# inferrna/Core

Hardware: AMD Instinct MI355X
Metric: Mrays/s (primary+shadow), 1M-tri scene (higher is better)
Workload: dtype f32

## Files before the change

core_amd/csrc/yk_device.hip:

```cpp
#include <hip/hip_runtime.h>

#include <algorithm>
#include <atomic>
#include <climits>
#include <chrono>
#include <cmath>
#include <cstdio>
#include <cstdlib>
#include <cstring>
#include <mutex>
#include <type_traits>
#include <stdexcept>
#include <string>
#include <thread>
#include <vector>

#include "../../include/yk_api.h"
#include "../../include/yk_test_hooks.h"
#include "../../include/yk_test_hooks_light.h"
#include "photon_map.h"
#include "scene.h"
#include "yk_internal.h"
#include "yk_math.h"

// ... 1780 lines not shown
  if (hit) s_q[off + __popcll(hm & ((1ull << lane) - 1ull))] = (int)threadIdx.x;
  __syncthreads();
  const bool valid = (int)threadIdx.x < tot;
  src = valid ? s_q[threadIdx.x] : 0;
  return valid;
}

enum : uint8_t { SL_TRACED = 1, SL_ADDS = 2 };
struct Batch;
__device__ __forceinline__ long long slot_of(const Batch& B, long long c, int k);
enum : int { PH_HIT = 1, PH_DIFFUSE = 2, PH_LIGHT = 4 };
enum : int { PS_ALIVE = 1, PS_RESOLVE = 2, PS_CONT = 4, PS_EST = 8, PS_EMIT = 256 };

struct Batch {
  int* prim_hit;
  unsigned* soffs;
  float* col;
  float* alpha;
  yk_ray* p_rays;
  yk_hit* p_hits;
  float* thr;
  float* pathcol;
  float* scol_next;
  float* wlast;
  float* emit_b;
  int* pstate;
  int* lsel;
  int* q_owner[2];
  yk_ray* q_rays[2];
  yk_hit* q_hits[2];
  float4* s_dir;
  int split;
  uint8_t* s_occl;
  unsigned* s_idx;
  float* sl_contrib;
  uint8_t* sl_flags;
  float4* samples;
  float2* sxy;
  char4* pext;
  int K;
  long long cap;
  long long kstride;
// ... 1 lines not shown
  long long slot_base;
  const unsigned long long* mq_words;
  int mq_region;
  unsigned* psample;
  uint8_t* incl;
  uint8_t* caus;
  float* emit0;
  int ts;
  float* s_filt;
  float* sl_aux;
};
__device__ __forceinline__ long long slot_of(const Batch& B, long long c, int k) {
  return B.slot_base + (long long)k * B.kstride + c;
}

struct RenderConst {
  int ps;
  int multipass;
  int pass_off;
  int spec;
  int trace_caustics;
  int rdepth;
  int level;
  int spp;
  int nsub;
  int bounces;
  int integrator;
  int transp_bg;
  int nlights;
  int has_bg;
// ... 51 lines not shown
    int lo = 0, hi = TL.ntiles - 1;
    while (lo < hi) {
      const int mid = (lo + hi + 1) >> 1;
      if (TL.base[mid] <= c) lo = mid;
      else hi = mid - 1;
    }
    const int4 T = TL.tiles[lo];
    const long long local = c - TL.base[lo];
    s = (int)((unsigned)local % (unsigned)R.spp);
    const int pl = (int)((unsigned)local / (unsigned)R.spp);
    j = T.x + pl % T.z;
    i = T.y + pl / T.z;
  }
  const unsigned so = fnv32a((unsigned)i * fnv32a((unsigned)j));
  const unsigned psample = (unsigned)(R.pass_off + s);
  B.soffs[c] = so;
  if (R.ps) B.psample[c] = psample;
  float dx = 0.5f, dy = 0.5f;
  if (R.multipass) {
    dx = ri_vdc(psample, so);
    dy = ri_s(psample, so);
  } else if (R.spp > 1) {
    dx = (0.5f + (float)s) * R.d1;
    dy = ri_lp((unsigned)s + so, 0u);
  }
  B.sxy[c] = make_float2(dx, dy);
  const float px = (float)j + dx, py = (float)i + dy;
  const v3 vr = ld3(c_cam.vright), vu = ld3(c_cam.vup), vt = ld3(c_cam.vto), cz = ld3(c_cam.camZ);
  v3 d = vadd(vadd(vmul(px, vr), vmul(py, vu)), vt);
  d = vnormalize_cam(d);
  const v3 from = ld3(c_cam.pos);
// ... 230 lines not shown
}

__device__ __forceinline__ void flush_shadow(const Batch& B, long long c, int kend, int nr, unsigned base,
                                             unsigned long long traced) {
  if (nr == 0) return;
  unsigned r = base;
  for (int k = 0; k < kend; ++k) {
    const long long slot = slot_of(B, c, k);
    const bool t = k < 64 ? ((traced >> k) & 1ull) != 0ull : (B.sl_flags[slot] & SL_TRACED) != 0;
    if (t) B.s_idx[r++] = B.split ? ((unsigned)k << B.kshift) | (unsigned)(B.slot_base + c) : (unsigned)slot;
  }
}

template <bool DIFF = false>
__device__ __forceinline__ yk_ray path_first_segment(const Batch& B, const RenderConst& R, long long c,
                                                     const SurfPt& sp, const DMat& M, v3 dir, int isub) {
  const unsigned s = R.ps ? B.psample[c] : (unsigned)c % (unsigned)R.spp;
  const unsigned offs = (unsigned)(R.nsub * (int)s) + B.soffs[c] + (unsigned)isub;
  const float s1 = ri_vdc(offs, 0u);
  const float s2 = (float)scr_halton(2, offs);
  float pdf, W = B.wlast[c];
  bool ok;
  v3 pdir = V3(0.f, 0.f, 0.f);
  c3 scol = mat_sample<DIFF>(M, sp, vneg(dir), pdir, s1, s2, BSDF_DIFFUSE | BSDF_REFLECT | BSDF_TRANSMIT, pdf, W, ok);
  B.wlast[c] = W;
  scol = cscale(W, scol);
  B.thr[3 * c] = scol.r;
  B.thr[3 * c + 1] = scol.g;
  B.thr[3 * c + 2] = scol.b;
  yk_ray r;
  put_ray(r, sp.P, pdir, YK_MIN_RAYDIST, -1.0f);
  return r;
}

template <bool DIFF, bool XL>
__global__ void __launch_bounds__(YK_PRIMARY_BLOCK) k_shade_primary(DScene S, Batch B, RenderConst R, long long nc,
                                                       unsigned long long* __restrict__ qword) {
  __shared__ DMat s_mats[kMaxMats];
  {
    const int nw = S.nmats * (int)(sizeof(DMat) / sizeof(int));
// ... 17 lines not shown
      const v3 from = V3(r.from[0], r.from[1], r.from[2]), dir = V3(r.dir[0], r.dir[1], r.dir[2]);
      const SurfPt sp = make_surface(S, from, dir, h);
      const DMat& M = s_mats[sp.mat];
      const v3 wo = vneg(dir);
      ph = PH_HIT;
      if (M.flags & BSDF_EMIT) {
        const c3 e = mat_emit(M, sp, wo, true);
        if (R.spec && R.integrator != YK_INTEGRATOR_PHOTON && M.type == YK_MAT_LIGHT) em = e;
        else col = cadd(col, e);
        if (R.integrator == YK_INTEGRATOR_PHOTON && !R.pm_showmap) col = cadd(col, mat_emit(M, sp, wo, false));
        if (M.type == YK_MAT_LIGHT) ph |= PH_LIGHT;
      }
      if (M.flags & BSDF_DIFFUSE) ph |= PH_DIFFUSE;
      if ((M.flags & BSDF_DIFFUSE) && !R.pm_showmap) {
        const unsigned s = R.ps ? B.psample[c] : (unsigned)c % (unsigned)R.spp;
        int k0 = 0;
        for (int l = 0; l < R.nlights; ++l) {
          nr += gen_light<DIFF, XL>(B, c, k0, l, sp, wo, s, B.soffs[c], (unsigned)l, traced, s_mats);
          k0 += c_lights[l].nslots;
        }
        kend = k0;
        if (nr) put_org(B, c, sp.P);
        if (R.integrator == YK_INTEGRATOR_PATH) {
          B.wlast[c] = 0.f;
          seg = path_first_segment<DIFF>(B, R, c, sp, M, dir, 0);
          emit = true;
          if (R.spec) {
            B.incl[c] = 0;
            B.caus[c] = 0;
          }
        }
      }
      alpha = 1.0f;
    } else if (R.has_bg) {
      col = cadd(col, C3(R.bg[0], R.bg[1], R.bg[2]));
    }
    B.prim_hit[c] = ph;
    B.col[3 * c] = col.r;
    B.col[3 * c + 1] = col.g;
    B.col[3 * c + 2] = col.b;
    B.alpha[c] = alpha;
    if (R.spec) {
      B.emit0[3 * c] = em.r;
      B.emit0[3 * c + 1] = em.g;
      B.emit0[3 * c + 2] = em.b;
    }
    if (!R.merged) {
      B.pathcol[3 * c] = 0.f;
      B.pathcol[3 * c + 1] = 0.f;
      B.pathcol[3 * c + 2] = 0.f;
    }
    if (!emit) B.wlast[c] = 0.f;
  }
  unsigned sbase, q;
  wave_append2<YK_PRIMARY_APPEND_WAVE>(qword, valid ? (unsigned)nr : 0u, emit ? 1u : 0u, sbase, q);
  if (valid) flush_shadow(B, c, kend, nr, sbase, traced);
  if (emit) {
    st_ray(&B.q_rays[1][q], seg);
    B.q_owner[1][q] = (int)c;
  }
}

__device__ __forceinline__ c3 slot_value_ts(const Batch& B, long long slot, int kind, c3 lcol, bool spot = false) {
  const c3 a = get_contrib(B, slot);
  const float4 x = *reinterpret_cast<const float4*>(B.sl_aux + 4 * slot);
  const c3 sc = C3(B.s_filt[3 * slot], B.s_filt[3 * slot + 1], B.s_filt[3 * slot + 2]);
  if (kind == 0) {
// ... 52 lines not shown
  B.col[3 * c + 2] = B.col[3 * c + 2] + dl.b;
}

template <bool DIFF>
__global__ void __launch_bounds__(YK_BOUNCE_BLOCK) k_path_start(DScene S, Batch B, RenderConst R, long long nc, int isub,
                                                    unsigned long long* __restrict__ qword) {
  const long long c = (long long)blockIdx.x * blockDim.x + threadIdx.x;
  const bool valid = c < nc;
  bool emit = false;
  yk_ray r;
  if (valid && (B.prim_hit[c] & PH_DIFFUSE)) {
    const yk_hit h = B.p_hits[c];
    const yk_ray pr = B.p_rays[c];
    const v3 from = V3(pr.from[0], pr.from[1], pr.from[2]), dir = V3(pr.dir[0], pr.dir[1], pr.dir[2]);
    const SurfPt sp = make_surface(S, from, dir, h);
    r = path_first_segment<DIFF>(B, R, c, sp, c_mats[sp.mat], dir, isub);
    emit = true;
    if (R.spec) {
      B.incl[c] = 0;
      B.caus[c] = 0;
    }
  }
  unsigned sbase, q;
  wave_append2<YK_BOUNCE_APPEND_WAVE>(qword, 0u, emit ? 1u : 0u, sbase, q);
  if (emit) {
    st_ray(&B.q_rays[1][q], r);
    B.q_owner[1][q] = (int)c;
  }
}

template <bool DIFF, bool XL>
// ... 6 lines not shown
  if (qb >= nq) return;
  unsigned qpre = 0;
  if (B.mq_words)
    for (int r = 0; r < B.mq_region; ++r) qpre += (unsigned)B.mq_words[r];
  long long qi = qb + threadIdx.x;
  bool valid = qi < nq;
  {
    const int prim = valid ? B.q_hits[qin][qi].prim : 0;
    if (valid && prim < 0) {
      const long long c = B.q_owner[qin][qi];
      if (R.spec && depth >= 2 && B.caus[c] && R.has_bg) {
        B.pathcol[3 * c] = B.pathcol[3 * c] + B.thr[3 * c] * R.bg[0];
        B.pathcol[3 * c + 1] = B.pathcol[3 * c + 1] + B.thr[3 * c + 1] * R.bg[1];
        B.pathcol[3 * c + 2] = B.pathcol[3 * c + 2] + B.thr[3 * c + 2] * R.bg[2];
      }
      B.pstate[c] = 0;
    }
    int src;
    valid = pack_block<bounce_block(DIFF)>(valid && prim >= 0, src);
    qi = qb + src;
  }
  const long long c = valid ? B.q_owner[qin][qi] : 0;
  int nr = 0, kend = 0;
  unsigned long long traced = 0;
  bool emit_next = false;
  yk_ray nxt;
  if (valid) {
    const yk_hit h = B.q_hits[qin][qi];
    {
      const yk_ray pr = B.q_rays[qin][qi];
      const v3 from = V3(pr.from[0], pr.from[1], pr.from[2]), dir = V3(pr.dir[0], pr.dir[1], pr.dir[2]);
      const SurfPt sp = make_surface(S, from, dir, h);
      const DMat& M = c_mats[sp.mat];
      const v3 pwo = vneg(dir);
      const unsigned s = R.ps ? B.psample[c] : (unsigned)c % (unsigned)R.spp;
      const unsigned offs = (unsigned)(R.nsub * (int)s) + B.soffs[c] + (unsigned)isub;
      int ps = PS_RESOLVE;
      if ((depth == 1 || (M.flags & BSDF_DIFFUSE)) && R.nlights > 0) {
        Halton h2;
        hal_start(h2, 2u, (unsigned)((int)offs - 1));
        int lnum = (int)(hal_next(h2) * (float)R.nlights);
        if (lnum > R.nlights - 1) lnum = R.nlights - 1;
        if (R.nlights == 1) nr = gen_light<DIFF, XL>(B, c, 0, 0, sp, pwo, s, B.soffs[c], 0u, traced);
        else nr = gen_light<DIFF, XL>(B, c, 0, lnum, sp, pwo, s, B.soffs[c], (unsigned)lnum, traced);
        kend = c_lights[lnum].nslots;
        if (nr) put_org(B, c, sp.P);
        if (R.nlights > 1) B.lsel[c] = lnum;
        ps |= PS_EST;
      }
      c3 em = C3(0.f, 0.f, 0.f);
      bool emits = false;
      if (depth == 1 && (M.flags & BSDF_EMIT)) {
        em = mat_emit(M, sp, pwo, false);
        emits = true;
      }
      if (R.spec && depth >= 2 && B.caus[c] && (M.flags & BSDF_SPECULAR)) {
        em = mat_emit(M, sp, pwo, true);
        emits = true;
      }
      if (emits) {
        B.emit_b[3 * c] = em.r;
        B.emit_b[3 * c + 1] = em.g;
        B.emit_b[3 * c + 2] = em.b;
        ps |= PS_EMIT;
      }
      if (depth < R.bounces) {
        const float s1 = (float)scr_halton(4 * depth + 3, offs);
        const float s2 = (float)scr_halton(4 * depth + 4, offs);
        float pdf, W = B.wlast[c];
        bool ok;
        v3 ndir = dir;
        unsigned sfl;
        c3 sc = mat_sample<DIFF>(M, sp, pwo, ndir, s1, s2, BSDF_ALL, pdf, W, ok, sfl);
        B.wlast[c] = W;
        sc = cscale(W, sc);
        if (!cblack(sc)) {
          if (R.spec) {
            const uint8_t caustic =
                (R.trace_caustics && (sfl & (BSDF_SPECULAR | BSDF_GLOSSY | BSDF_FILTER))) ? 1 : 0;
            B.caus[c] = caustic;
            B.incl[c] = caustic;
          }
          put_ray(nxt, sp.P, ndir, YK_MIN_RAYDIST, -1.0f);
          emit_next = true;
          B.scol_next[3 * c] = sc.r;
          B.scol_next[3 * c + 1] = sc.g;
          B.scol_next[3 * c + 2] = sc.b;
          ps |= PS_CONT;
        }
      }
      B.pstate[c] = ps;
    }
  }
  unsigned sbase, qn;
  wave_append2<YK_BOUNCE_APPEND_WAVE>(qword, valid ? (unsigned)nr : 0u, emit_next ? 1u : 0u, sbase, qn);
  if (valid) flush_shadow(B, c, kend, nr, sbase + qpre, traced);
  if (emit_next) {
    st_ray(&B.q_rays[qin ^ 1][qn], nxt);
    B.q_owner[qin ^ 1][qn] = (int)c;
  }
}

inline auto shade_primary_fn(bool diff, bool xl) {
  return xl ? (diff ? k_shade_primary<true, true> : k_shade_primary<false, true>)
            : (diff ? k_shade_primary<true, false> : k_shade_primary<false, false>);
}
inline auto shade_bounce_fn(bool diff, bool xl) {
  return xl ? (diff ? k_shade_bounce<true, true> : k_shade_bounce<false, true>)
            : (diff ? k_shade_bounce<true, false> : k_shade_bounce<false, false>);
}

__global__ void __launch_bounds__(256) k_resolve_bounce(Batch B, RenderConst R,
                                                        const unsigned long long* __restrict__ qin_word, int depth,
                                                        int qin) {
  const long long nq = (long long)(*qin_word >> 32);
  const long long qi = (long long)blockIdx.x * blockDim.x + threadIdx.x;
  if (qi >= nq) return;
  const long long c = B.q_owner[qin][qi];
  const int ps = B.pstate[c];
  if (!(ps & PS_RESOLVE)) return;
  c3 lcol = C3(0.f, 0.f, 0.f);
  if (ps & PS_EST) {
    const int lnum = R.nlights > 1 ? B.lsel[c] : 0;
    lcol = cscale((float)R.nlights, resolve_light(B, c, 0, lnum));
  }
  if ((depth == 1 || R.spec) && (ps & PS_EMIT))
    lcol = cadd(lcol, C3(B.emit_b[3 * c], B.emit_b[3 * c + 1], B.emit_b[3 * c + 2]));
  const c3 thr = C3(B.thr[3 * c], B.thr[3 * c + 1], B.thr[3 * c + 2]);
  B.pathcol[3 * c] = B.pathcol[3 * c] + lcol.r * thr.r;
  B.pathcol[3 * c + 1] = B.pathcol[3 * c + 1] + lcol.g * thr.g;
  B.pathcol[3 * c + 2] = B.pathcol[3 * c + 2] + lcol.b * thr.b;
  if (ps & PS_CONT) {
    B.thr[3 * c] = thr.r * B.scol_next[3 * c];
    B.thr[3 * c + 1] = thr.g * B.scol_next[3 * c + 1];
    B.thr[3 * c + 2] = thr.b * B.scol_next[3 * c + 2];
    B.pstate[c] = PS_ALIVE;
  } else {
    B.pstate[c] = 0;
  }
}


__host__ __device__ inline Batch merged_region(Batch B, int depth) {
  B.slot_base = (long long)depth * B.cap;
  B.mq_region = depth;
  if (depth >= 1) {
    const long long o = (long long)(depth - 1) * B.cap;
    B.pstate += o;
    B.lsel += o;
    B.emit_b += 3 * o;
    B.scol_next += 3 * o;
  }
  return B;
}

__global__ void __launch_bounds__(256) k_resolve_merged(Batch B, RenderConst R, long long nc, int bounces) {
  const long long c = (long long)blockIdx.x * blockDim.x + threadIdx.x;
  if (c >= nc) return;
  c3 col = C3(B.col[3 * c], B.col[3 * c + 1], B.col[3 * c + 2]);
  if (!(B.prim_hit[c] & PH_DIFFUSE)) {
    B.samples[c] = make_float4(col.r, col.g, col.b, B.alpha[c]);
    return;
  }
  {
    c3 dl = C3(0.f, 0.f, 0.f);
    int k0 = 0;
    for (int l = 0; l < R.nlights; ++l) {
      dl = cadd(dl, resolve_light(B, c, k0, l));
      k0 += c_lights[l].nslots;
    }
    col = C3(col.r + dl.r, col.g + dl.g, col.b + dl.b);
  }
  c3 thr = C3(B.thr[3 * c], B.thr[3 * c + 1], B.thr[3 * c + 2]);
  c3 pc = C3(0.f, 0.f, 0.f);
  for (int depth = 1; depth <= bounces; ++depth) {
    const Batch Bd = merged_region(B, depth);
    const int ps = Bd.pstate[c];
    if (!(ps & PS_RESOLVE)) break;
    c3 lcol = C3(0.f, 0.f, 0.f);
    if (ps & PS_EST) {
      const int lnum = R.nlights > 1 ? Bd.lsel[c] : 0;
      lcol = cscale((float)R.nlights, resolve_light(Bd, c, 0, lnum));
    }
    if (depth == 1 && (ps & PS_EMIT))
      lcol = cadd(lcol, C3(Bd.emit_b[3 * c], Bd.emit_b[3 * c + 1], Bd.emit_b[3 * c + 2]));
    pc = C3(pc.r + lcol.r * thr.r, pc.g + lcol.g * thr.g, pc.b + lcol.b * thr.b);
    if (!(ps & PS_CONT)) break;
    thr = C3(thr.r * Bd.scol_next[3 * c], thr.g * Bd.scol_next[3 * c + 1], thr.b * Bd.scol_next[3 * c + 2]);
  }
  const float ns = (float)R.nsub;
  col = cadd(col, C3(pc.r / ns, pc.g / ns, pc.b / ns));
  B.samples[c] = make_float4(col.r, col.g, col.b, B.alpha[c]);
}

__global__ void __launch_bounds__(256) k_finish(Batch B, RenderConst R, long long nc) {
  const long long c = (long long)blockIdx.x * blockDim.x + threadIdx.x;
  if (c >= nc) return;
  c3 col = C3(B.col[3 * c], B.col[3 * c + 1], B.col[3 * c + 2]);
  if (R.integrator == YK_INTEGRATOR_PATH && (B.prim_hit[c] & PH_DIFFUSE)) {
    const float ns = (float)R.nsub;
    col = cadd(col, C3(B.pathcol[3 * c] / ns, B.pathcol[3 * c + 1] / ns, B.pathcol[3 * c + 2] / ns));
  }
  B.samples[c] = make_float4(col.r, col.g, col.b, B.alpha[c]);
// ... 6 lines not shown
  float* E;
  float* D;
  float* P;
  int* flags;
  int* child;
  float* rcol;
  float* alpha;
  yk_ray* ray;
  unsigned* soffs;
  unsigned* psample;
  unsigned long long* count;
  long long cap;
  int* overflow;
  float* malpha;
};

__global__ void __launch_bounds__(256) k_finish_spec(Batch B, RenderConst R, NodeStore NS, long long base,
                                                     long long n) {
  const long long i = (long long)blockIdx.x * blockDim.x + threadIdx.x;
  if (i >= n) return;
  const long long node = base + i;
  const int ph = B.prim_hit[i];
  const bool loop = R.integrator == YK_INTEGRATOR_PATH && (ph & PH_DIFFUSE);
  c3 P = C3(0.f, 0.f, 0.f);
  if (loop) {
    const float ns = (float)R.nsub;
    P = C3(B.pathcol[3 * i] / ns, B.pathcol[3 * i + 1] / ns, B.pathcol[3 * i + 2] / ns);
  }
  int f = 0;
  if (ph & PH_HIT) f |= NF_HIT;
// ... 40 lines not shown
  mat_specular(M, sp, vneg(dir), refl, refr, d, col);
  const bool want[2] = {refl, refr};
#pragma unroll
  for (int k = 0; k < 2; ++k) {
    if (!want[k]) continue;
    const unsigned long long id = atomicAdd(NS.count, 1ull);
    if ((long long)id >= NS.cap) {
      *NS.overflow = 1;
      continue;
    }
    NS.child[2 * node + k] = (int)id;
    NS.rcol[6 * node + 3 * k] = col[k].r;
    NS.rcol[6 * node + 3 * k + 1] = col[k].g;
    NS.rcol[6 * node + 3 * k + 2] = col[k].b;
    put_ray(NS.ray[id], sp.P, d[k], YK_MIN_RAYDIST, -1.0f);
    NS.soffs[id] = B.soffs[i];
    NS.psample[id] = B.psample[i];
  }
}

__global__ void __launch_bounds__(256) k_fold(Batch B, RenderConst R, NodeStore NS, long long nc) {
  const long long c = (long long)blockIdx.x * blockDim.x + threadIdx.x;
  if (c >= nc) return;
  constexpr int kMaxLevel = 22;
  int nodes[kMaxLevel], stage[kMaxLevel];
  c3 acc[kMaxLevel];
  float alp[kMaxLevel];
  const bool pt = R.integrator == YK_INTEGRATOR_PATH, pm = R.integrator == YK_INTEGRATOR_PHOTON;
  const float a_init = R.transp_bg ? 0.f : 1.f;
  float result_alpha = 0.f;
  bool e = true;
// ... 313 lines not shown
  DBuf() = default;
  DBuf(const DBuf&) = delete;
  DBuf& operator=(const DBuf&) = delete;
  ~DBuf() { release(); }
};

}

struct Pipe {
  hipStream_t stream = nullptr;
  hipEvent_t ev0 = nullptr, ev1 = nullptr;
  DBuf<unsigned long long> counters;
  DBuf<unsigned long long> words;
  DBuf<uint2> ovf;
  std::vector<hipEvent_t> evpool;
  DBuf<unsigned> soffs, s_idx;
  DBuf<float> col, alpha, thr, pathcol, scol_next, wlast, emit_b, sl_contrib;
  DBuf<int> prim_hit, pstate, lsel, qo0, qo1, tile_base;
  DBuf<int4> tiles;
  DBuf<yk_ray> p_rays, qr0, qr1;
  DBuf<float4> s_dir;
  DBuf<yk_hit> p_hits, qh0, qh1;
  DBuf<uint8_t> sl_flags, s_occl;
  DBuf<float4> samples;
  DBuf<float2> sxy;
  DBuf<char4> pext;
  DBuf<unsigned> psample;
  DBuf<uint8_t> incl, caus;
  DBuf<float> emit0;
  DBuf<float> fgl, fglen;
  DBuf<float4> lkq;
  DBuf<float> s_filt, sl_aux;
  void create() {
// ... 7 lines not shown
      hipEvent_t e;
      HIPCHK(hipEventCreate(&e));
      evpool.push_back(e);
    }
    return evpool[i];
  }
  ~Pipe() {
    for (auto e : evpool) (void)hipEventDestroy(e);
    if (ev0) (void)hipEventDestroy(ev0);
    if (ev1) (void)hipEventDestroy(ev1);
    if (stream) (void)hipStreamDestroy(stream);
  }
  template <class T>
  static long long held(const DBuf<T>& b) { return (long long)(b.n * sizeof(T)); }
  long long batch_bytes() const {
    return held(soffs) + held(s_idx) + held(col) + held(alpha) + held(thr) + held(pathcol) + held(scol_next) +
           held(wlast) + held(emit_b) + held(sl_contrib) + held(prim_hit) + held(pstate) + held(lsel) + held(qo0) +
           held(qo1) + held(tile_base) + held(tiles) + held(p_rays) + held(qr0) + held(qr1) + held(s_dir) +
           held(p_hits) + held(qh0) + held(qh1) + held(sl_flags) + held(s_occl) + held(samples) + held(sxy) +
           held(pext) + held(psample) + held(incl) + held(caus) + held(emit0) + held(fgl) + held(fglen) + held(lkq) +
           held(s_filt) + held(sl_aux);
  }
  long long all_bytes() const { return batch_bytes() + held(counters) + held(words) + held(ovf); }
  Batch bind(long long maxc, int K, int tiles_per_batch, bool spec, bool ts, int regions, bool split) {
    const long long nst = std::max(1, regions - 1);
    soffs.ensure(maxc);
    col.ensure(3 * maxc);
    alpha.ensure(maxc);
    prim_hit.ensure(maxc);
    p_rays.ensure(maxc);
    p_hits.ensure(maxc);
    thr.ensure(3 * maxc);
    pathcol.ensure(3 * maxc);
    scol_next.ensure(3 * maxc * nst);
    wlast.ensure(maxc);
    emit_b.ensure(3 * maxc * nst);
    pstate.ensure(maxc * nst);
    lsel.ensure(maxc * nst);
    qo0.ensure(maxc);
    qo1.ensure(maxc);
    qr0.ensure(maxc);
    qr1.ensure(maxc);
    qh0.ensure(maxc);
    qh1.ensure(maxc);
    s_dir.ensure(maxc * (split ? K + 1 : 2 * K) * regions);
    s_occl.ensure(maxc * K * regions);
    s_idx.ensure(maxc * K * regions);
    sl_contrib.ensure(3 * maxc * K * regions);
    sl_flags.ensure(maxc * K * regions);
    samples.ensure(maxc);
    sxy.ensure(maxc);
    pext.ensure(maxc);
    tiles.ensure(tiles_per_batch);
    tile_base.ensure(tiles_per_batch + 1);
    Batch B{};
    B.prim_hit = prim_hit.p;
    B.soffs = soffs.p;
    B.col = col.p;
    B.alpha = alpha.p;
    B.p_rays = p_rays.p;
    B.p_hits = p_hits.p;
    B.thr = thr.p;
    B.pathcol = pathcol.p;
    B.scol_next = scol_next.p;
    B.wlast = wlast.p;
    B.emit_b = emit_b.p;
    B.pstate = pstate.p;
    B.lsel = lsel.p;
    B.q_owner[0] = qo0.p;
    B.q_owner[1] = qo1.p;
    B.q_rays[0] = qr0.p;
    B.q_rays[1] = qr1.p;
    B.q_hits[0] = qh0.p;
    B.q_hits[1] = qh1.p;
    B.s_dir = s_dir.p;
    B.s_occl = s_occl.p;
    B.s_idx = s_idx.p;
    B.sl_contrib = sl_contrib.p;
    B.sl_flags = sl_flags.p;
    B.samples = samples.p;
    B.sxy = sxy.p;
    B.pext = pext.p;
    B.split = split ? 1 : 0;
// ... 1410 lines not shown
      long long g0 = 0, g1 = nc;
      for (int level = 1; level <= spec_levels; ++level) {
        unsigned long long cnt = 0;
        HIPCHK(hipMemcpyAsync(&cnt, NS.count, sizeof cnt, hipMemcpyDeviceToHost, P.stream));
        HIPCHK(hipStreamSynchronize(P.stream));
        if ((long long)cnt > NS.cap) return set_error(YK_ERR_INTERNAL, "specular node store overflow");
        g0 = g1;
        g1 = (long long)cnt;
        if (g1 <= g0) break;
        RenderConst Rl = R;
        Rl.level = level;
        for (long long off = g0; off < g1; off += maxc) {
          const long long n = std::min<long long>(maxc, g1 - off);
          Batch Bc = B;
          Bc.p_rays = NS.ray + off;
          Bc.soffs = NS.soffs + off;
          Bc.psample = NS.psample + off;
          shade_entries(Bc, Rl, n, off);
        }
      }
      hipLaunchKernelGGL(k_fold, dim3(grid_for(nc)), dim3(256), 0, P.stream, B, R, NS, nc);
      HIPCHK(hipGetLastError());
    }
    if (!d->spec) {
    trace(true, ray_src(B.p_rays), nullptr, RayCount{nullptr, 0, nc}, B.p_hits, nullptr);
    hipLaunchKernelGGL(shade_primary_fn(d->diff_only, d->xl_lights), dim3(grid_for(nc, YK_PRIMARY_BLOCK)), dim3(YK_PRIMARY_BLOCK), 0, P.stream, d->S, B, R, nc, qw(0, 0));
    HIPCHK(hipGetLastError());
    if (!merged) {
      trace(false, shadow_src(B), B.s_idx, RayCount{qw(0, 0), 0, 0}, nullptr, B.s_occl);
      hipLaunchKernelGGL(k_resolve_primary, dim3(grid_for(nc)), dim3(256), 0, P.stream, B, R, nc);
      HIPCHK(hipGetLastError());
    }
// ... 345 lines not shown
```

core_amd/csrc/yk_photon.inc:

```

struct PMapDev {
  const uint2* nodes;
  const float4* pos;
  const float4* dir;
  const float4* col;
  int n;
  const uint4* pk;
};

constexpr int kPStack = 48;
constexpr int kMaxSearch = 256;

struct ScratchStack {
  uint2 s[kPStack];
  __device__ __forceinline__ void put(int i, uint2 e) { s[i] = e; }
  __device__ __forceinline__ uint2 get(int i) const { return s[i]; }
};
constexpr int kLdsPStack = 16;
struct LdsStack {
  uint2* base;
  int lane, stride;
  __device__ __forceinline__ void put(int i, uint2 e) { base[i * stride + lane] = e; }
  __device__ __forceinline__ uint2 get(int i) const { return base[i * stride + lane]; }
};
// ... 482 lines not shown
enum : int { FG_ADD = 16, FG_EMIT = 32, FG_CAUS = 64, FG_SPECF = 128 };

template <bool DIFF>
__global__ void __launch_bounds__(YK_APPEND_BLOCK) k_fg_start(DScene S, Batch B, RenderConst R, long long nc, int isub,
                                                  float* __restrict__ fg_lcol, unsigned long long* __restrict__ qword) {
  const long long c = (long long)blockIdx.x * blockDim.x + threadIdx.x;
  const bool valid = c < nc;
  bool emit = false;
  yk_ray r;
  if (valid && (B.prim_hit[c] & PH_DIFFUSE)) {
    const yk_hit h = B.p_hits[c];
    const yk_ray pr = B.p_rays[c];
    const v3 from = V3(pr.from[0], pr.from[1], pr.from[2]), dir = V3(pr.dir[0], pr.dir[1], pr.dir[2]);
    const SurfPt sp = make_surface(S, from, dir, h);
    const unsigned s = R.ps ? B.psample[c] : (unsigned)c % (unsigned)R.spp;
    const unsigned offs = (unsigned)(R.nsub * (int)s) + B.soffs[c] + (unsigned)isub;
    const float s1 = ri_vdc(offs, 0u);
    const float s2 = (float)scr_halton(2, offs);
    float pdf, W = B.wlast[c];
    bool ok;
    v3 pdir = V3(0.f, 0.f, 0.f);
    c3 scol = mat_sample<DIFF>(c_mats[sp.mat], sp, vneg(dir), pdir, s1, s2, BSDF_DIFFUSE | BSDF_REFLECT | BSDF_TRANSMIT,
                               pdf, W, ok);
    B.wlast[c] = W;
    scol = C3(scol.r * W, scol.g * W, scol.b * W);
    B.pstate[c] = 0;
    if (!cblack(scol)) {
      B.thr[3 * c] = scol.r;
      B.thr[3 * c + 1] = scol.g;
      B.thr[3 * c + 2] = scol.b;
      fg_lcol[3 * c] = 0.f;
      fg_lcol[3 * c + 1] = 0.f;
      fg_lcol[3 * c + 2] = 0.f;
      put_ray(r, sp.P, pdir, YK_MIN_RAYDIST, -1.0f);
      emit = true;
    }
  }
  unsigned sb, q;
  wave_append2<YK_PM_APPEND_WAVE>(qword, 0u, emit ? 1u : 0u, sb, q);
  if (emit) {
    B.q_rays[1][q] = r;
// ... 8 lines not shown
__global__ void __launch_bounds__(YK_APPEND_BLOCK) __attribute__((amdgpu_waves_per_eu(DIFF ? YK_FG_WAVES_D : 1)))
k_fg_hit(DScene S, Batch B, RenderConst R, PMConst PM,
                                                const unsigned long long* __restrict__ qin_word, int it, int isub,
                                                int qin, float* __restrict__ fg_lcol, float* __restrict__ fg_len,
                                                unsigned long long* __restrict__ qword, float4* __restrict__ lq,
                                                unsigned long long* __restrict__ lword) {
  const long long nq = (long long)(*qin_word >> 32);
  const long long qb = (long long)blockIdx.x * blockDim.x;
  if (qb >= nq) return;
  const long long qi = qb + threadIdx.x;
  bool valid = qi < nq;
  {
    const int prim = valid ? B.q_hits[qin][qi].prim : 0;
    if (valid && prim < 0) {
      const long long c = B.q_owner[qin][qi];
      if (it > 0 && (B.pstate[c] & FG_CAUS) && R.has_bg) {
        B.pathcol[3 * c] = B.pathcol[3 * c] + B.thr[3 * c] * R.bg[0];
        B.pathcol[3 * c + 1] = B.pathcol[3 * c + 1] + B.thr[3 * c + 1] * R.bg[1];
        B.pathcol[3 * c + 2] = B.pathcol[3 * c + 2] + B.thr[3 * c + 2] * R.bg[2];
      }
      B.pstate[c] = 0;
    }
    valid = valid && prim >= 0;
  }
  const long long c = valid ? B.q_owner[qin][qi] : 0;
  int nr = 0, kend = 0;
  unsigned long long traced = 0;
  bool emit_next = false;
  yk_ray nxt;
  bool look = false;
  v3 lp = V3(0.f, 0.f, 0.f), ln = lp;
  if (valid) {
    const yk_hit h = B.q_hits[qin][qi];
    int ps = B.pstate[c];
    bool caustic = (ps & FG_CAUS) != 0;
    {
      const yk_ray pr = B.q_rays[qin][qi];
      const v3 from = V3(pr.from[0], pr.from[1], pr.from[2]), dir = V3(pr.dir[0], pr.dir[1], pr.dir[2]);
      const SurfPt sp = make_surface(S, from, dir, h);
      const DMat& M = c_mats[sp.mat];
      float length;
      bool do_bounce;
      if (it == 0) {
        length = h.t;
        caustic = false;
        do_bounce = (length < PM.gather_dist) || (M.flags & BSDF_SPECULAR);
      } else {
        length = fg_len[c] + h.t;
        caustic = (caustic || it == 1) && (ps & FG_SPECF);
        do_bounce = caustic || (length < PM.gather_dist);
      }
      const bool close = length < PM.gather_dist;
      fg_len[c] = length;
      ps = PS_RESOLVE | (caustic ? FG_CAUS : 0);
      const v3 pwo = vneg(dir);
      if (it < PM.fg_bounces && do_bounce) {
        const unsigned s = R.ps ? B.psample[c] : (unsigned)c % (unsigned)R.spp;
        const unsigned offs = (unsigned)(R.nsub * (int)s) + B.soffs[c] + (unsigned)isub;
        if (M.flags & BSDF_DIFFUSE) {
          if (close) {
            if (R.nlights > 0) {
              Halton h2;
              hal_start(h2, 2u, (unsigned)((int)offs - 1));
              int lnum = (int)(hal_next(h2) * (float)R.nlights);
              if (lnum > R.nlights - 1) lnum = R.nlights - 1;
              nr = gen_light<DIFF>(B, c, 0, lnum, sp, pwo, s, B.soffs[c], (unsigned)lnum, traced);
              kend = c_lights[lnum].nslots;
              if (nr) put_org(B, c, sp.P);
              B.lsel[c] = lnum;
              ps |= PS_EST;
            } else {
              fg_lcol[3 * c] = 0.f;
              fg_lcol[3 * c + 1] = 0.f;
              fg_lcol[3 * c + 2] = 0.f;
            }
          } else if (caustic) {
            look = true;
            lp = sp.P;
            ln = face_forward(sp.Ng, sp.N, pwo);
          }
          if (close || caustic) {
            ps |= FG_ADD;
            if (M.flags & BSDF_EMIT) {
              const c3 em = mat_emit(M, sp, pwo, false);
              B.emit_b[3 * c] = em.r;
              B.emit_b[3 * c + 1] = em.g;
              B.emit_b[3 * c + 2] = em.b;
              ps |= FG_EMIT;
            }
          }
        }
        const int d4 = 4 * it;
        const float s1 = (float)scr_halton(d4 + 3, offs);
        const float s2 = (float)scr_halton(d4 + 4, offs);
        float pdf, W = B.wlast[c];
        bool ok;
        v3 ndir = dir;
        unsigned sfl;
        const unsigned fl = close ? BSDF_ALL : (BSDF_SPECULAR | BSDF_REFLECT | BSDF_TRANSMIT | BSDF_FILTER);
        c3 sc = mat_sample<DIFF>(M, sp, pwo, ndir, s1, s2, fl, pdf, W, ok, sfl);
        B.wlast[c] = W;
        if (pdf > 1.0e-6f) {
          sc = C3(sc.r * W, sc.g * W, sc.b * W);
          B.scol_next[3 * c] = sc.r;
          B.scol_next[3 * c + 1] = sc.g;
          B.scol_next[3 * c + 2] = sc.b;
          if (sfl & (BSDF_SPECULAR | BSDF_FILTER)) ps |= FG_SPECF;
          put_ray(nxt, sp.P, ndir, YK_MIN_RAYDIST, -1.0f);
          emit_next = true;
          ps |= PS_CONT;
        }
      } else if (M.flags & (BSDF_DIFFUSE | BSDF_GLOSSY)) {
        look = true;
        lp = sp.P;
        ln = face_forward(sp.Ng, sp.N, pwo);
        ps |= FG_ADD;
        if (M.flags & BSDF_EMIT) {
          const c3 em = mat_emit(M, sp, pwo, false);
          B.emit_b[3 * c] = em.r;
          B.emit_b[3 * c + 1] = em.g;
          B.emit_b[3 * c + 2] = em.b;
          ps |= FG_EMIT;
        }
      }
      B.pstate[c] = ps;
    }
  }
  unsigned sbase, qn;
  wave_append2<YK_PM_APPEND_WAVE>(qword, valid ? (unsigned)nr : 0u, emit_next ? 1u : 0u, sbase, qn);
  if (valid) flush_shadow(B, c, kend, nr, sbase, traced);
  if (emit_next) {
    B.q_rays[qin ^ 1][qn] = nxt;
    B.q_owner[qin ^ 1][qn] = (int)c;
  }
  unsigned lb, lb_hi;
  if (!YK_PM_APPEND_WAVE) __syncthreads();
  wave_append2<YK_PM_APPEND_WAVE>(lword, look ? 1u : 0u, 0u, lb, lb_hi);
  if (look) {
    lq[2 * (size_t)lb] = make_float4(lp.x, lp.y, lp.z, __int_as_float((int)c));
    lq[2 * (size_t)lb + 1] = make_float4(ln.x, ln.y, ln.z, 0.f);
// ... 77 lines not shown
        fg_lcol[3 * (size_t)c + 1] = pc.y;
        fg_lcol[3 * (size_t)c + 2] = pc.z;
      }
      c = -1;
    }
  }
}

__global__ void __launch_bounds__(256) k_fg_resolve(Batch B, RenderConst R,
                                                    const unsigned long long* __restrict__ qin_word, int qin,
                                                    float* __restrict__ fg_lcol) {
  const long long nq = (long long)(*qin_word >> 32);
  const long long qi = (long long)blockIdx.x * blockDim.x + threadIdx.x;
  if (qi >= nq) return;
  const long long c = B.q_owner[qin][qi];
  const int ps = B.pstate[c];
  if (!(ps & PS_RESOLVE)) return;
  c3 lcol = C3(fg_lcol[3 * c], fg_lcol[3 * c + 1], fg_lcol[3 * c + 2]);
  if (ps & PS_EST) lcol = cscale((float)R.nlights, resolve_light(B, c, 0, B.lsel[c]));
  if (ps & FG_ADD) {
    if (ps & FG_EMIT) lcol = cadd(lcol, C3(B.emit_b[3 * c], B.emit_b[3 * c + 1], B.emit_b[3 * c + 2]));
    const c3 thr = C3(B.thr[3 * c], B.thr[3 * c + 1], B.thr[3 * c + 2]);
    B.pathcol[3 * c] = B.pathcol[3 * c] + lcol.r * thr.r;
    B.pathcol[3 * c + 1] = B.pathcol[3 * c + 1] + lcol.g * thr.g;
    B.pathcol[3 * c + 2] = B.pathcol[3 * c + 2] + lcol.b * thr.b;
  }
  fg_lcol[3 * c] = lcol.r;
  fg_lcol[3 * c + 1] = lcol.g;
  fg_lcol[3 * c + 2] = lcol.b;
  if (ps & PS_CONT) {
    B.thr[3 * c] = B.thr[3 * c] * B.scol_next[3 * c];
    B.thr[3 * c + 1] = B.thr[3 * c + 1] * B.scol_next[3 * c + 1];
    B.thr[3 * c + 2] = B.thr[3 * c + 2] * B.scol_next[3 * c + 2];
    B.pstate[c] = ps & (FG_CAUS | FG_SPECF);
  } else {
    B.pstate[c] = 0;
  }
}

__device__ __forceinline__ c3 caustic_estimate(const DScene& S, const Batch& B, const PMConst& PM, long long c) {
  const yk_ray r = B.p_rays[c];
  const v3 from = V3(r.from[0], r.from[1], r.from[2]), dir = V3(r.dir[0], r.dir[1], r.dir[2]);
  const SurfPt sp = make_surface(S, from, dir, B.p_hits[c]);
  const v3 wo = vneg(dir);
  PFound f[kMaxSearch];
  float g = PM.caus_radius * PM.caus_radius;
  const int ng = pm_gather(PM.cmap, sp.P, f, PM.caustic_mix, g);
  g = 1.f / g;
  c3 sum = C3(0.f, 0.f, 0.f);
  if (ng > 0) {
    const DMat& M = c_mats[sp.mat];
// ... 37 lines not shown
```

Measured before the change: 3501.

## Pack per-path bounce state into float4/uint2 structs for vectorized access

Merges the separate SoA arrays (scol_next, pstate, emit_b, lsel, soffs, wlast) into packed records: cont (throughput scale plus state), emis (emission plus selected light), and samp (sample offset plus weight). Bounce, resolve and merge kernels now do one 16-byte load or store per record instead of several scattered scalar accesses, cutting memory transactions on the gather-by-owner paths. In exchange, node shading needs an extra small kernel to repack soffs into samp, and state-only updates now write into a wider record.

```diff
diff --git a/core_amd/csrc/yk_device.hip b/core_amd/csrc/yk_device.hip
--- a/core_amd/csrc/yk_device.hip
+++ b/core_amd/csrc/yk_device.hip
@@ -1818,18 +1818,15 @@
 
 struct Batch {
   int* prim_hit;
-  unsigned* soffs;
+  uint2* samp;
   float* col;
   float* alpha;
   yk_ray* p_rays;
   yk_hit* p_hits;
   float* thr;
   float* pathcol;
-  float* scol_next;
-  float* wlast;
-  float* emit_b;
-  int* pstate;
-  int* lsel;
+  float4* cont;
+  float4* emis;
   int* q_owner[2];
   yk_ray* q_rays[2];
   yk_hit* q_hits[2];
@@ -1861,6 +1858,18 @@
   return B.slot_base + (long long)k * B.kstride + c;
 }
 
+__device__ __forceinline__ void put_cont(const Batch& B, long long c, c3 scol, int ps) {
+  B.cont[c] = make_float4(scol.r, scol.g, scol.b, __int_as_float(ps));
+}
+__device__ __forceinline__ void put_pstate(const Batch& B, long long c, int ps) { B.cont[c].w = __int_as_float(ps); }
+__device__ __forceinline__ int get_pstate(const Batch& B, long long c) { return __float_as_int(B.cont[c].w); }
+__device__ __forceinline__ void put_emit(const Batch& B, long long c, c3 em) {
+  const float x[3] = {em.r, em.g, em.b};
+  __builtin_memcpy(&B.emis[c], x, 12);
+}
+__device__ __forceinline__ void put_lsel(const Batch& B, long long c, int lnum) { B.emis[c].w = __int_as_float(lnum); }
+__device__ __forceinline__ void put_wlast(const Batch& B, long long c, float W) { B.samp[c].y = __float_as_uint(W); }
+
 struct RenderConst {
   int ps;
   int multipass;
@@ -1942,7 +1951,7 @@
   }
   const unsigned so = fnv32a((unsigned)i * fnv32a((unsigned)j));
   const unsigned psample = (unsigned)(R.pass_off + s);
-  B.soffs[c] = so;
+  B.samp[c] = make_uint2(so, 0u);
   if (R.ps) B.psample[c] = psample;
   float dx = 0.5f, dy = 0.5f;
   if (R.multipass) {
@@ -2203,16 +2212,17 @@
 
 template <bool DIFF = false>
 __device__ __forceinline__ yk_ray path_first_segment(const Batch& B, const RenderConst& R, long long c,
-                                                     const SurfPt& sp, const DMat& M, v3 dir, int isub) {
+                                                     const SurfPt& sp, const DMat& M, v3 dir, int isub,
+                                                     unsigned soffs, float W) {
   const unsigned s = R.ps ? B.psample[c] : (unsigned)c % (unsigned)R.spp;
-  const unsigned offs = (unsigned)(R.nsub * (int)s) + B.soffs[c] + (unsigned)isub;
+  const unsigned offs = (unsigned)(R.nsub * (int)s) + soffs + (unsigned)isub;
   const float s1 = ri_vdc(offs, 0u);
   const float s2 = (float)scr_halton(2, offs);
-  float pdf, W = B.wlast[c];
+  float pdf;
   bool ok;
   v3 pdir = V3(0.f, 0.f, 0.f);
   c3 scol = mat_sample<DIFF>(M, sp, vneg(dir), pdir, s1, s2, BSDF_DIFFUSE | BSDF_REFLECT | BSDF_TRANSMIT, pdf, W, ok);
-  B.wlast[c] = W;
+  put_wlast(B, c, W);
   scol = cscale(W, scol);
   B.thr[3 * c] = scol.r;
   B.thr[3 * c + 1] = scol.g;
@@ -2260,16 +2270,16 @@
       if (M.flags & BSDF_DIFFUSE) ph |= PH_DIFFUSE;
       if ((M.flags & BSDF_DIFFUSE) && !R.pm_showmap) {
         const unsigned s = R.ps ? B.psample[c] : (unsigned)c % (unsigned)R.spp;
+        const unsigned soffs = B.samp[c].x;
         int k0 = 0;
         for (int l = 0; l < R.nlights; ++l) {
-          nr += gen_light<DIFF, XL>(B, c, k0, l, sp, wo, s, B.soffs[c], (unsigned)l, traced, s_mats);
+          nr += gen_light<DIFF, XL>(B, c, k0, l, sp, wo, s, soffs, (unsigned)l, traced, s_mats);
           k0 += c_lights[l].nslots;
         }
         kend = k0;
         if (nr) put_org(B, c, sp.P);
         if (R.integrator == YK_INTEGRATOR_PATH) {
-          B.wlast[c] = 0.f;
-          seg = path_first_segment<DIFF>(B, R, c, sp, M, dir, 0);
+          seg = path_first_segment<DIFF>(B, R, c, sp, M, dir, 0, soffs, 0.f);
           emit = true;
           if (R.spec) {
             B.incl[c] = 0;
@@ -2296,7 +2306,6 @@
       B.pathcol[3 * c + 1] = 0.f;
       B.pathcol[3 * c + 2] = 0.f;
     }
-    if (!emit) B.wlast[c] = 0.f;
   }
   unsigned sbase, q;
   wave_append2<YK_PRIMARY_APPEND_WAVE>(qword, valid ? (unsigned)nr : 0u, emit ? 1u : 0u, sbase, q);
@@ -2379,7 +2388,8 @@
     const yk_ray pr = B.p_rays[c];
     const v3 from = V3(pr.from[0], pr.from[1], pr.from[2]), dir = V3(pr.dir[0], pr.dir[1], pr.dir[2]);
     const SurfPt sp = make_surface(S, from, dir, h);
-    r = path_first_segment<DIFF>(B, R, c, sp, c_mats[sp.mat], dir, isub);
+    const uint2 sr = B.samp[c];
+    r = path_first_segment<DIFF>(B, R, c, sp, c_mats[sp.mat], dir, isub, sr.x, __uint_as_float(sr.y));
     emit = true;
     if (R.spec) {
       B.incl[c] = 0;
@@ -2416,7 +2426,7 @@
         B.pathcol[3 * c + 1] = B.pathcol[3 * c + 1] + B.thr[3 * c + 1] * R.bg[1];
         B.pathcol[3 * c + 2] = B.pathcol[3 * c + 2] + B.thr[3 * c + 2] * R.bg[2];
       }
-      B.pstate[c] = 0;
+      put_cont(B, c, C3(0.f, 0.f, 0.f), 0);
     }
     int src;
     valid = pack_block<bounce_block(DIFF)>(valid && prim >= 0, src);
@@ -2436,18 +2446,19 @@
       const DMat& M = c_mats[sp.mat];
       const v3 pwo = vneg(dir);
       const unsigned s = R.ps ? B.psample[c] : (unsigned)c % (unsigned)R.spp;
-      const unsigned offs = (unsigned)(R.nsub * (int)s) + B.soffs[c] + (unsigned)isub;
+      const uint2 sr = B.samp[c];
+      const unsigned offs = (unsigned)(R.nsub * (int)s) + sr.x + (unsigned)isub;
       int ps = PS_RESOLVE;
       if ((depth == 1 || (M.flags & BSDF_DIFFUSE)) && R.nlights > 0) {
         Halton h2;
         hal_start(h2, 2u, (unsigned)((int)offs - 1));
         int lnum = (int)(hal_next(h2) * (float)R.nlights);
         if (lnum > R.nlights - 1) lnum = R.nlights - 1;
-        if (R.nlights == 1) nr = gen_light<DIFF, XL>(B, c, 0, 0, sp, pwo, s, B.soffs[c], 0u, traced);
-        else nr = gen_light<DIFF, XL>(B, c, 0, lnum, sp, pwo, s, B.soffs[c], (unsigned)lnum, traced);
+        if (R.nlights == 1) nr = gen_light<DIFF, XL>(B, c, 0, 0, sp, pwo, s, sr.x, 0u, traced);
+        else nr = gen_light<DIFF, XL>(B, c, 0, lnum, sp, pwo, s, sr.x, (unsigned)lnum, traced);
         kend = c_lights[lnum].nslots;
         if (nr) put_org(B, c, sp.P);
-        if (R.nlights > 1) B.lsel[c] = lnum;
+        if (R.nlights > 1) put_lsel(B, c, lnum);
         ps |= PS_EST;
       }
       c3 em = C3(0.f, 0.f, 0.f);
@@ -2461,20 +2472,19 @@
         emits = true;
       }
       if (emits) {
-        B.emit_b[3 * c] = em.r;
-        B.emit_b[3 * c + 1] = em.g;
-        B.emit_b[3 * c + 2] = em.b;
+        put_emit(B, c, em);
         ps |= PS_EMIT;
       }
+      c3 sc = C3(0.f, 0.f, 0.f);
       if (depth < R.bounces) {
         const float s1 = (float)scr_halton(4 * depth + 3, offs);
         const float s2 = (float)scr_halton(4 * depth + 4, offs);
-        float pdf, W = B.wlast[c];
+        float pdf, W = __uint_as_float(sr.y);
         bool ok;
         v3 ndir = dir;
         unsigned sfl;
-        c3 sc = mat_sample<DIFF>(M, sp, pwo, ndir, s1, s2, BSDF_ALL, pdf, W, ok, sfl);
-        B.wlast[c] = W;
+        sc = mat_sample<DIFF>(M, sp, pwo, ndir, s1, s2, BSDF_ALL, pdf, W, ok, sfl);
+        put_wlast(B, c, W);
         sc = cscale(W, sc);
         if (!cblack(sc)) {
           if (R.spec) {
@@ -2485,13 +2495,10 @@
           }
           put_ray(nxt, sp.P, ndir, YK_MIN_RAYDIST, -1.0f);
           emit_next = true;
-          B.scol_next[3 * c] = sc.r;
-          B.scol_next[3 * c + 1] = sc.g;
-          B.scol_next[3 * c + 2] = sc.b;
           ps |= PS_CONT;
         }
       }
-      B.pstate[c] = ps;
+      put_cont(B, c, sc, ps);
     }
   }
   unsigned sbase, qn;
@@ -2519,26 +2526,26 @@
   const long long qi = (long long)blockIdx.x * blockDim.x + threadIdx.x;
   if (qi >= nq) return;
   const long long c = B.q_owner[qin][qi];
-  const int ps = B.pstate[c];
+  const float4 cr = B.cont[c];
+  const int ps = __float_as_int(cr.w);
   if (!(ps & PS_RESOLVE)) return;
+  const bool adds_em = (depth == 1 || R.spec) && (ps & PS_EMIT), picks = (ps & PS_EST) && R.nlights > 1;
+  float4 er = make_float4(0.f, 0.f, 0.f, 0.f);
+  if (adds_em || picks) er = B.emis[c];
   c3 lcol = C3(0.f, 0.f, 0.f);
-  if (ps & PS_EST) {
-    const int lnum = R.nlights > 1 ? B.lsel[c] : 0;
-    lcol = cscale((float)R.nlights, resolve_light(B, c, 0, lnum));
-  }
-  if ((depth == 1 || R.spec) && (ps & PS_EMIT))
-    lcol = cadd(lcol, C3(B.emit_b[3 * c], B.emit_b[3 * c + 1], B.emit_b[3 * c + 2]));
+  if (ps & PS_EST) lcol = cscale((float)R.nlights, resolve_light(B, c, 0, picks ? __float_as_int(er.w) : 0));
+  if (adds_em) lcol = cadd(lcol, C3(er.x, er.y, er.z));
   const c3 thr = C3(B.thr[3 * c], B.thr[3 * c + 1], B.thr[3 * c + 2]);
   B.pathcol[3 * c] = B.pathcol[3 * c] + lcol.r * thr.r;
   B.pathcol[3 * c + 1] = B.pathcol[3 * c + 1] + lcol.g * thr.g;
   B.pathcol[3 * c + 2] = B.pathcol[3 * c + 2] + lcol.b * thr.b;
   if (ps & PS_CONT) {
-    B.thr[3 * c] = thr.r * B.scol_next[3 * c];
-    B.thr[3 * c + 1] = thr.g * B.scol_next[3 * c + 1];
-    B.thr[3 * c + 2] = thr.b * B.scol_next[3 * c + 2];
-    B.pstate[c] = PS_ALIVE;
+    B.thr[3 * c] = thr.r * cr.x;
+    B.thr[3 * c + 1] = thr.g * cr.y;
+    B.thr[3 * c + 2] = thr.b * cr.z;
+    put_pstate(B, c, PS_ALIVE);
   } else {
-    B.pstate[c] = 0;
+    put_pstate(B, c, 0);
   }
 }
 
@@ -2548,10 +2555,8 @@
   B.mq_region = depth;
   if (depth >= 1) {
     const long long o = (long long)(depth - 1) * B.cap;
-    B.pstate += o;
-    B.lsel += o;
-    B.emit_b += 3 * o;
-    B.scol_next += 3 * o;
+    B.cont += o;
+    B.emis += o;
   }
   return B;
 }
@@ -2577,18 +2582,18 @@
   c3 pc = C3(0.f, 0.f, 0.f);
   for (int depth = 1; depth <= bounces; ++depth) {
     const Batch Bd = merged_region(B, depth);
-    const int ps = Bd.pstate[c];
+    const float4 cr = Bd.cont[c];
+    const int ps = __float_as_int(cr.w);
     if (!(ps & PS_RESOLVE)) break;
+    const bool adds_em = depth == 1 && (ps & PS_EMIT), picks = (ps & PS_EST) && R.nlights > 1;
+    float4 er = make_float4(0.f, 0.f, 0.f, 0.f);
+    if (adds_em || picks) er = Bd.emis[c];
     c3 lcol = C3(0.f, 0.f, 0.f);
-    if (ps & PS_EST) {
-      const int lnum = R.nlights > 1 ? Bd.lsel[c] : 0;
-      lcol = cscale((float)R.nlights, resolve_light(Bd, c, 0, lnum));
-    }
-    if (depth == 1 && (ps & PS_EMIT))
-      lcol = cadd(lcol, C3(Bd.emit_b[3 * c], Bd.emit_b[3 * c + 1], Bd.emit_b[3 * c + 2]));
+    if (ps & PS_EST) lcol = cscale((float)R.nlights, resolve_light(Bd, c, 0, picks ? __float_as_int(er.w) : 0));
+    if (adds_em) lcol = cadd(lcol, C3(er.x, er.y, er.z));
     pc = C3(pc.r + lcol.r * thr.r, pc.g + lcol.g * thr.g, pc.b + lcol.b * thr.b);
     if (!(ps & PS_CONT)) break;
-    thr = C3(thr.r * Bd.scol_next[3 * c], thr.g * Bd.scol_next[3 * c + 1], thr.b * Bd.scol_next[3 * c + 2]);
+    thr = C3(thr.r * cr.x, thr.g * cr.y, thr.b * cr.z);
   }
   const float ns = (float)R.nsub;
   col = cadd(col, C3(pc.r / ns, pc.g / ns, pc.b / ns));
@@ -2625,6 +2630,12 @@
   int* overflow;
   float* malpha;
 };
+
+__global__ void __launch_bounds__(256) k_node_samp(uint2* __restrict__ samp, const unsigned* __restrict__ soffs,
+                                                   long long n) {
+  const long long i = (long long)blockIdx.x * blockDim.x + threadIdx.x;
+  if (i < n) samp[i] = make_uint2(soffs[i], 0u);
+}
 
 __global__ void __launch_bounds__(256) k_finish_spec(Batch B, RenderConst R, NodeStore NS, long long base,
                                                      long long n) {
@@ -2695,7 +2706,7 @@
     NS.rcol[6 * node + 3 * k + 1] = col[k].g;
     NS.rcol[6 * node + 3 * k + 2] = col[k].b;
     put_ray(NS.ray[id], sp.P, d[k], YK_MIN_RAYDIST, -1.0f);
-    NS.soffs[id] = B.soffs[i];
+    NS.soffs[id] = B.samp[i].x;
     NS.psample[id] = B.psample[i];
   }
 }
@@ -3039,9 +3050,11 @@
   DBuf<unsigned long long> words;
   DBuf<uint2> ovf;
   std::vector<hipEvent_t> evpool;
-  DBuf<unsigned> soffs, s_idx;
-  DBuf<float> col, alpha, thr, pathcol, scol_next, wlast, emit_b, sl_contrib;
-  DBuf<int> prim_hit, pstate, lsel, qo0, qo1, tile_base;
+  DBuf<unsigned> s_idx;
+  DBuf<uint2> samp;
+  DBuf<float4> cont, emis;
+  DBuf<float> col, alpha, thr, pathcol, sl_contrib;
+  DBuf<int> prim_hit, qo0, qo1, tile_base;
   DBuf<int4> tiles;
   DBuf<yk_ray> p_rays, qr0, qr1;
   DBuf<float4> s_dir;
@@ -3079,8 +3092,8 @@
   template <class T>
   static long long held(const DBuf<T>& b) { return (long long)(b.n * sizeof(T)); }
   long long batch_bytes() const {
-    return held(soffs) + held(s_idx) + held(col) + held(alpha) + held(thr) + held(pathcol) + held(scol_next) +
-           held(wlast) + held(emit_b) + held(sl_contrib) + held(prim_hit) + held(pstate) + held(lsel) + held(qo0) +
+    return held(samp) + held(s_idx) + held(col) + held(alpha) + held(thr) + held(pathcol) + held(cont) +
+           held(emis) + held(sl_contrib) + held(prim_hit) + held(qo0) +
            held(qo1) + held(tile_base) + held(tiles) + held(p_rays) + held(qr0) + held(qr1) + held(s_dir) +
            held(p_hits) + held(qh0) + held(qh1) + held(sl_flags) + held(s_occl) + held(samples) + held(sxy) +
            held(pext) + held(psample) + held(incl) + held(caus) + held(emit0) + held(fgl) + held(fglen) + held(lkq) +
@@ -3089,7 +3102,7 @@
   long long all_bytes() const { return batch_bytes() + held(counters) + held(words) + held(ovf); }
   Batch bind(long long maxc, int K, int tiles_per_batch, bool spec, bool ts, int regions, bool split) {
     const long long nst = std::max(1, regions - 1);
-    soffs.ensure(maxc);
+    samp.ensure(maxc);
     col.ensure(3 * maxc);
     alpha.ensure(maxc);
     prim_hit.ensure(maxc);
@@ -3097,11 +3110,8 @@
     p_hits.ensure(maxc);
     thr.ensure(3 * maxc);
     pathcol.ensure(3 * maxc);
-    scol_next.ensure(3 * maxc * nst);
-    wlast.ensure(maxc);
-    emit_b.ensure(3 * maxc * nst);
-    pstate.ensure(maxc * nst);
-    lsel.ensure(maxc * nst);
+    cont.ensure(maxc * nst);
+    emis.ensure(maxc * nst);
     qo0.ensure(maxc);
     qo1.ensure(maxc);
     qr0.ensure(maxc);
@@ -3120,18 +3130,15 @@
     tile_base.ensure(tiles_per_batch + 1);
     Batch B{};
     B.prim_hit = prim_hit.p;
-    B.soffs = soffs.p;
+    B.samp = samp.p;
     B.col = col.p;
     B.alpha = alpha.p;
     B.p_rays = p_rays.p;
     B.p_hits = p_hits.p;
     B.thr = thr.p;
     B.pathcol = pathcol.p;
-    B.scol_next = scol_next.p;
-    B.wlast = wlast.p;
-    B.emit_b = emit_b.p;
-    B.pstate = pstate.p;
-    B.lsel = lsel.p;
+    B.cont = cont.p;
+    B.emis = emis.p;
     B.q_owner[0] = qo0.p;
     B.q_owner[1] = qo1.p;
     B.q_rays[0] = qr0.p;
@@ -4572,8 +4579,9 @@
           const long long n = std::min<long long>(maxc, g1 - off);
           Batch Bc = B;
           Bc.p_rays = NS.ray + off;
-          Bc.soffs = NS.soffs + off;
           Bc.psample = NS.psample + off;
+          hipLaunchKernelGGL(k_node_samp, dim3(grid_for(n)), dim3(256), 0, P.stream, Bc.samp, NS.soffs + off, n);
+          HIPCHK(hipGetLastError());
           shade_entries(Bc, Rl, n, off);
         }
       }
diff --git a/core_amd/csrc/yk_photon.inc b/core_amd/csrc/yk_photon.inc
--- a/core_amd/csrc/yk_photon.inc
+++ b/core_amd/csrc/yk_photon.inc
@@ -520,17 +520,18 @@
     const v3 from = V3(pr.from[0], pr.from[1], pr.from[2]), dir = V3(pr.dir[0], pr.dir[1], pr.dir[2]);
     const SurfPt sp = make_surface(S, from, dir, h);
     const unsigned s = R.ps ? B.psample[c] : (unsigned)c % (unsigned)R.spp;
-    const unsigned offs = (unsigned)(R.nsub * (int)s) + B.soffs[c] + (unsigned)isub;
+    const uint2 sr = B.samp[c];
+    const unsigned offs = (unsigned)(R.nsub * (int)s) + sr.x + (unsigned)isub;
     const float s1 = ri_vdc(offs, 0u);
     const float s2 = (float)scr_halton(2, offs);
-    float pdf, W = B.wlast[c];
+    float pdf, W = __uint_as_float(sr.y);
     bool ok;
     v3 pdir = V3(0.f, 0.f, 0.f);
     c3 scol = mat_sample<DIFF>(c_mats[sp.mat], sp, vneg(dir), pdir, s1, s2, BSDF_DIFFUSE | BSDF_REFLECT | BSDF_TRANSMIT,
                                pdf, W, ok);
-    B.wlast[c] = W;
+    put_wlast(B, c, W);
     scol = C3(scol.r * W, scol.g * W, scol.b * W);
-    B.pstate[c] = 0;
+    put_pstate(B, c, 0);
     if (!cblack(scol)) {
       B.thr[3 * c] = scol.r;
       B.thr[3 * c + 1] = scol.g;
@@ -569,12 +570,12 @@
     const int prim = valid ? B.q_hits[qin][qi].prim : 0;
     if (valid && prim < 0) {
       const long long c = B.q_owner[qin][qi];
-      if (it > 0 && (B.pstate[c] & FG_CAUS) && R.has_bg) {
+      if (it > 0 && (get_pstate(B, c) & FG_CAUS) && R.has_bg) {
         B.pathcol[3 * c] = B.pathcol[3 * c] + B.thr[3 * c] * R.bg[0];
         B.pathcol[3 * c + 1] = B.pathcol[3 * c + 1] + B.thr[3 * c + 1] * R.bg[1];
         B.pathcol[3 * c + 2] = B.pathcol[3 * c + 2] + B.thr[3 * c + 2] * R.bg[2];
       }
-      B.pstate[c] = 0;
+      put_pstate(B, c, 0);
     }
     valid = valid && prim >= 0;
   }
@@ -587,8 +588,9 @@
   v3 lp = V3(0.f, 0.f, 0.f), ln = lp;
   if (valid) {
     const yk_hit h = B.q_hits[qin][qi];
-    int ps = B.pstate[c];
+    int ps = get_pstate(B, c);
     bool caustic = (ps & FG_CAUS) != 0;
+    c3 sc = C3(0.f, 0.f, 0.f);
     {
       const yk_ray pr = B.q_rays[qin][qi];
       const v3 from = V3(pr.from[0], pr.from[1], pr.from[2]), dir = V3(pr.dir[0], pr.dir[1], pr.dir[2]);
@@ -611,7 +613,8 @@
       const v3 pwo = vneg(dir);
       if (it < PM.fg_bounces && do_bounce) {
         const unsigned s = R.ps ? B.psample[c] : (unsigned)c % (unsigned)R.spp;
-        const unsigned offs = (unsigned)(R.nsub * (int)s) + B.soffs[c] + (unsigned)isub;
+        const uint2 sr = B.samp[c];
+        const unsigned offs = (unsigned)(R.nsub * (int)s) + sr.x + (unsigned)isub;
         if (M.flags & BSDF_DIFFUSE) {
           if (close) {
             if (R.nlights > 0) {
@@ -619,10 +622,10 @@
               hal_start(h2, 2u, (unsigned)((int)offs - 1));
               int lnum = (int)(hal_next(h2) * (float)R.nlights);
               if (lnum > R.nlights - 1) lnum = R.nlights - 1;
-              nr = gen_light<DIFF>(B, c, 0, lnum, sp, pwo, s, B.soffs[c], (unsigned)lnum, traced);
+              nr = gen_light<DIFF>(B, c, 0, lnum, sp, pwo, s, sr.x, (unsigned)lnum, traced);
               kend = c_lights[lnum].nslots;
               if (nr) put_org(B, c, sp.P);
-              B.lsel[c] = lnum;
+              put_lsel(B, c, lnum);
               ps |= PS_EST;
             } else {
               fg_lcol[3 * c] = 0.f;
@@ -637,10 +640,7 @@
           if (close || caustic) {
             ps |= FG_ADD;
             if (M.flags & BSDF_EMIT) {
-              const c3 em = mat_emit(M, sp, pwo, false);
-              B.emit_b[3 * c] = em.r;
-              B.emit_b[3 * c + 1] = em.g;
-              B.emit_b[3 * c + 2] = em.b;
+              put_emit(B, c, mat_emit(M, sp, pwo, false));
               ps |= FG_EMIT;
             }
           }
@@ -648,18 +648,15 @@
         const int d4 = 4 * it;
         const float s1 = (float)scr_halton(d4 + 3, offs);
         const float s2 = (float)scr_halton(d4 + 4, offs);
-        float pdf, W = B.wlast[c];
+        float pdf, W = __uint_as_float(sr.y);
         bool ok;
         v3 ndir = dir;
         unsigned sfl;
         const unsigned fl = close ? BSDF_ALL : (BSDF_SPECULAR | BSDF_REFLECT | BSDF_TRANSMIT | BSDF_FILTER);
-        c3 sc = mat_sample<DIFF>(M, sp, pwo, ndir, s1, s2, fl, pdf, W, ok, sfl);
-        B.wlast[c] = W;
+        sc = mat_sample<DIFF>(M, sp, pwo, ndir, s1, s2, fl, pdf, W, ok, sfl);
+        put_wlast(B, c, W);
         if (pdf > 1.0e-6f) {
           sc = C3(sc.r * W, sc.g * W, sc.b * W);
-          B.scol_next[3 * c] = sc.r;
-          B.scol_next[3 * c + 1] = sc.g;
-          B.scol_next[3 * c + 2] = sc.b;
           if (sfl & (BSDF_SPECULAR | BSDF_FILTER)) ps |= FG_SPECF;
           put_ray(nxt, sp.P, ndir, YK_MIN_RAYDIST, -1.0f);
           emit_next = true;
@@ -671,14 +668,11 @@
         ln = face_forward(sp.Ng, sp.N, pwo);
         ps |= FG_ADD;
         if (M.flags & BSDF_EMIT) {
-          const c3 em = mat_emit(M, sp, pwo, false);
-          B.emit_b[3 * c] = em.r;
-          B.emit_b[3 * c + 1] = em.g;
-          B.emit_b[3 * c + 2] = em.b;
+          put_emit(B, c, mat_emit(M, sp, pwo, false));
           ps |= FG_EMIT;
         }
       }
-      B.pstate[c] = ps;
+      put_cont(B, c, sc, ps);
     }
   }
   unsigned sbase, qn;
@@ -786,12 +780,15 @@
   const long long qi = (long long)blockIdx.x * blockDim.x + threadIdx.x;
   if (qi >= nq) return;
   const long long c = B.q_owner[qin][qi];
-  const int ps = B.pstate[c];
+  const float4 cr = B.cont[c];
+  const int ps = __float_as_int(cr.w);
   if (!(ps & PS_RESOLVE)) return;
+  float4 er = make_float4(0.f, 0.f, 0.f, 0.f);
+  if (ps & (PS_EST | FG_EMIT)) er = B.emis[c];
   c3 lcol = C3(fg_lcol[3 * c], fg_lcol[3 * c + 1], fg_lcol[3 * c + 2]);
-  if (ps & PS_EST) lcol = cscale((float)R.nlights, resolve_light(B, c, 0, B.lsel[c]));
+  if (ps & PS_EST) lcol = cscale((float)R.nlights, resolve_light(B, c, 0, __float_as_int(er.w)));
   if (ps & FG_ADD) {
-    if (ps & FG_EMIT) lcol = cadd(lcol, C3(B.emit_b[3 * c], B.emit_b[3 * c + 1], B.emit_b[3 * c + 2]));
+    if (ps & FG_EMIT) lcol = cadd(lcol, C3(er.x, er.y, er.z));
     const c3 thr = C3(B.thr[3 * c], B.thr[3 * c + 1], B.thr[3 * c + 2]);
     B.pathcol[3 * c] = B.pathcol[3 * c] + lcol.r * thr.r;
     B.pathcol[3 * c + 1] = B.pathcol[3 * c + 1] + lcol.g * thr.g;
@@ -801,12 +798,12 @@
   fg_lcol[3 * c + 1] = lcol.g;
   fg_lcol[3 * c + 2] = lcol.b;
   if (ps & PS_CONT) {
-    B.thr[3 * c] = B.thr[3 * c] * B.scol_next[3 * c];
-    B.thr[3 * c + 1] = B.thr[3 * c + 1] * B.scol_next[3 * c + 1];
-    B.thr[3 * c + 2] = B.thr[3 * c + 2] * B.scol_next[3 * c + 2];
-    B.pstate[c] = ps & (FG_CAUS | FG_SPECF);
+    B.thr[3 * c] = B.thr[3 * c] * cr.x;
+    B.thr[3 * c + 1] = B.thr[3 * c + 1] * cr.y;
+    B.thr[3 * c + 2] = B.thr[3 * c + 2] * cr.z;
+    put_pstate(B, c, ps & (FG_CAUS | FG_SPECF));
   } else {
-    B.pstate[c] = 0;
+    put_pstate(B, c, 0);
   }
 }
 
```

Measured after the change: 3506 (median of 6 runs). About the same (+0.1%).
